# tnestmeyer/reflectance-filtering

Measured on AMD Instinct MI355X. Metric: megapixels/sec joint-bilateral sigma_c=20 sigma_s=22 @1080p, higher is better.
Workload: dtype f32

## Files before the change

reflectance_filtering_amd/csrc/rf_api.hip:

```cpp
#include "rf_common.hpp"

#include <atomic>
#include <cstring>

#include "reflectance_filtering_debug.h"

namespace rf {

void jbf_shutdown();
void cnn_shutdown();
void gf_shutdown();

char *last_error_buf()
{
    static thread_local char buf[512] = "";
    return buf;
}

int fail(int code, const char *fmt, ...)
{
    va_list ap;
    va_start(ap, fmt);
    vsnprintf(last_error_buf(), 512, fmt, ap);
    va_end(ap);
    return code;
}

static std::atomic<int> g_debug[kDbgCount];

int debug_get(int id) { return g_debug[id].load(std::memory_order_relaxed); }

}

extern "C" int rf_debug_option(const char *name, int value)
{
    static const char *const names[] = {"gf_two_kernel",     "jbf_stage_only",
                                                      "jbf_compiler_loop", "jbf_tile64_only",
                                                      "jbf_tune",          "jbf_f32_untiled",
                                                      "cnn_lds_columns",   "gf_seg_rows",
                                                      "gf_one_stream",     "gf_force_two_streams",
                                                      "gf_guide_cache",    "gf_chained",        "gf_no_compact",
                                                      "gf_exp_skip",       "gf_stagger",        "gf_parts",
                                                      "gf_s1_cap",         "gf_s1_min_wgs",
                                                      "jbf_lookahead1",    "gf_s1_legacy_strips",
                                                      "gf_exact_all_flagged", "gf_cw_chan_run",   "gf_exact"};
    static_assert(sizeof(names) / sizeof(names[0]) == rf::kDbgCount, "one name per DebugOption");
    if (name)
        for (int i = 0; i < rf::kDbgCount; i++)
            if (std::strcmp(name, names[i]) == 0)
                return rf::g_debug[i].exchange(value < 0 ? 0 : value);
    return rf::fail(RF_E_BADARG, "rf_debug_option: unknown option '%s'", name ? name : "(null)");
}

__global__ void clock_probe_kernel(unsigned long long *out, unsigned long long ticks)
{
    if (threadIdx.x != 0)
        return;
    const unsigned long long r0 = __builtin_amdgcn_s_memrealtime();
    const unsigned long long c0 = __builtin_amdgcn_s_memtime();
    unsigned long long r1 = r0;
    while (r1 - r0 < ticks) {
        __builtin_amdgcn_s_sleep(64);
        r1 = __builtin_amdgcn_s_memrealtime();
    }
    const unsigned long long c1 = __builtin_amdgcn_s_memtime();
    r1 = __builtin_amdgcn_s_memrealtime();
    out[0] = c1 - c0;
    out[1] = r1 - r0;
}

extern "C" int rf_debug_clock_probe(unsigned long long *out2, int micros, void *stream)
{
    if (!out2 || micros < 1 || micros > 1000000)
        return rf::fail(RF_E_BADARG, "rf_debug_clock_probe: bad argument");
    hipLaunchKernelGGL(clock_probe_kernel, dim3(1), dim3(64), 0, (hipStream_t)stream, out2,
                       (unsigned long long)micros * 100ull);
    RF_HIP_CHECK(hipGetLastError());
    return RF_OK;
}

#ifdef RF_GF_DEV_ONLY
extern "C" int rf_version(void) { return RF_VERSION | 0x40000000; }
#else
extern "C" int rf_version(void) { return RF_VERSION; }
#endif

#ifndef RF_TOOLCHAIN
#define RF_TOOLCHAIN "unknown toolchain"
#endif
extern "C" const char *rf_debug_build_info(void) { return RF_TOOLCHAIN; }

extern "C" const char *rf_last_error(void) { return rf::last_error_buf(); }

extern "C" int rf_shutdown(void)
{
    rf::jbf_shutdown();
    rf::cnn_shutdown();
    rf::gf_shutdown();
    return RF_OK;
}
```

reflectance_filtering_amd/csrc/rf_common.hpp:

```cpp
#pragma once
#include <hip/hip_runtime.h>

#include <cstdarg>
#include <cstdint>
#include <cstdio>

#include "reflectance_filtering.h"

namespace rf {

char *last_error_buf();
int fail(int code, const char *fmt, ...);

#define RF_HIP_CHECK(expr)                                                                   \
    do {                                                                                     \
        hipError_t _e = (expr);                                                              \
        if (_e != hipSuccess)                                                                \
            return ::rf::fail(RF_E_HIP, "%s failed: %s (%s:%d)", #expr, hipGetErrorString(_e), \
                              __FILE__, __LINE__);                                           \
    } while (0)

__host__ __device__ inline int border_interpolate(int p, int len, int border)
{
    if ((unsigned)p < (unsigned)len)
        return p;
    if (border == RF_BORDER_REPLICATE)
        return p < 0 ? 0 : len - 1;
    if (border == RF_BORDER_REFLECT || border == RF_BORDER_REFLECT_101) {
        const int delta = border == RF_BORDER_REFLECT_101;
        if (len == 1)
            return 0;
        do {
            p = p < 0 ? -p - 1 + delta : len - 1 - (p - len) - delta;
        } while ((unsigned)p >= (unsigned)len);
        return p;
    }
    if (border == RF_BORDER_WRAP) {
        if (p < 0)
            p -= ((p - len + 1) / len) * len;
        if (p >= len)
            p %= len;
        return p;
    }
    return -1;
}

__device__ inline uint8_t saturate_u8(float v)
{
    if (!(fabsf(v) < 2147483648.0f))
        return 0;
    int iv = __float2int_rn(v);
    iv = iv < 0 ? 0 : (iv > 255 ? 255 : iv);
    return (uint8_t)iv;
}

inline int ceil_div(int a, int b) { return (a + b - 1) / b; }

inline bool ranges_overlap(const void *a, size_t na, const void *b, size_t nb)
{
    const uintptr_t a0 = (uintptr_t)a, b0 = (uintptr_t)b;
    return a0 < b0 + nb && b0 < a0 + na;
}

enum DebugOption {
    kDbgGfTwoKernel = 0,
    kDbgJbfStageOnly,
    kDbgJbfCompilerLoop,
    kDbgJbfTile64Only,
    kDbgJbfTune,
    kDbgJbfF32Untiled,
    kDbgCnnLdsColumns,
    kDbgGfSegRows,
    kDbgGfOneStream,
    kDbgGfForceTwoStreams,
    kDbgGfGuideCache,
    kDbgGfChained,
    kDbgGfNoCompact,
    kDbgGfExpSkip,
    kDbgGfStagger,
    kDbgGfParts,
    kDbgGfS1Cap,
    kDbgGfS1MinWgs,
    kDbgJbfLookahead1,
    kDbgGfS1LegacyStrips,
    kDbgGfExactAllFlagged,
    kDbgGfCwChanRun,
    kDbgGfExact,
    kDbgCount
};
int debug_get(int id);

}
```

reflectance_filtering_amd/csrc/rf_jbf.hip:

```cpp
#include <atomic>
#include <cfloat>
#include <cmath>
#include <cstring>
#include <memory>
#include <mutex>
#include <type_traits>
#include <vector>

#include "rf_jbf_common.hpp"

namespace rf {

int jbf_colour_lut(int joint_cn, double sigma_color, std::vector<float> &lut)
{
    const double gauss_color_coeff = -0.5 / (sigma_color * sigma_color);
    const int nlut = 256 * joint_cn;
    lut.assign(nlut, 0.0f);
    for (int i = 0; i < nlut; i++)
        lut[i] = (float)std::exp(i * i * gauss_color_coeff);
    for (int i = 0; i < nlut; i++)
        if (lut[i] == 0.0f)
            return i + 1;
    return nlut;
}

void jbf_space_taps(int radius, double sigma_space, std::vector<int> &di, std::vector<int> &dj,
                    std::vector<float> &sw, std::vector<int> &hw)
{
    const double gauss_space_coeff = -0.5 / (sigma_space * sigma_space);
    di.clear();
    dj.clear();
    sw.clear();
    hw.assign(2 * radius + 1, -1);
    for (int i = -radius; i <= radius; i++)
        for (int j = -radius; j <= radius; j++) {
            double r = std::sqrt((double)i * i + (double)j * j);
            if (r > radius)
                continue;
            float wgt = (float)std::exp(r * r * gauss_space_coeff);
            di.push_back(i);
            dj.push_back(j);
            sw.push_back(wgt);
            if (j >= 0 && j > hw[i + radius])
                hw[i + radius] = j;
        }
}

namespace {

constexpr int kTileW = 64;
constexpr int kPix = 4;
constexpr int kMaxLds = 160 * 1024;
constexpr int kTlw2 = 144;
constexpr int kJbfMaxTiledR4 = 468;
constexpr int kJbfStageOnly = 0x1000, kJbfCompilerLoop = 0x2000, kJbfTile64Only = 0x4000;
constexpr int kJbfLookahead1 = 0x8000;

typedef uint32_t uint2v __attribute__((ext_vector_type(2)));
typedef float float4v __attribute__((ext_vector_type(4)));

struct JbfTables {
    int device = -1;
    int radius = 0;
    int joint_cn = 0;
    double sigma_color = 0, sigma_space = 0;
    int maxk = 0;
    int lut_len = 0;
    float *d_lut = nullptr;
    int *d_di = nullptr;
    int *d_dj = nullptr;
    float *d_sw = nullptr;
    int *d_hw = nullptr;
    int r4 = 0, sw_len = 0;
    float *d_swsym = nullptr;
    std::shared_ptr<void> keep;
};

struct CaptureRelax {
    hipStreamCaptureMode mode = hipStreamCaptureModeRelaxed;
    bool ok;
    CaptureRelax() { ok = hipThreadExchangeStreamCaptureMode(&mode) == hipSuccess; }
    ~CaptureRelax()
    {
        if (ok)
            (void)hipThreadExchangeStreamCaptureMode(&mode);
    }
};

struct JbfTableOwner {
    int device = 0;
    void *d_arena = nullptr;
    size_t bytes = 0;
    std::atomic<bool> pinned{false};
    ~JbfTableOwner()
    {
        int cur = 0;
        const bool switched = hipGetDevice(&cur) == hipSuccess && cur != device &&
                              hipSetDevice(device) == hipSuccess;
        if (d_arena)
            (void)hipFree(d_arena);
        if (switched)
            (void)hipSetDevice(cur);
    }
};

std::mutex g_mu;
std::vector<JbfTables> g_tables;
std::vector<std::shared_ptr<void>> g_retired;

bool stream_is_capturing(hipStream_t stream)
{
    hipStreamCaptureStatus cs = hipStreamCaptureStatusNone;
    if (hipStreamIsCapturing(stream, &cs) != hipSuccess) {
        (void)hipGetLastError();
        return false;
    }
    return cs != hipStreamCaptureStatusNone;
}

void drain_retired(hipStream_t stream)
{
    if (stream_is_capturing(stream))
        return;
    std::vector<std::shared_ptr<void>> bin;
    {
        std::lock_guard<std::mutex> lock(g_mu);
        bin.swap(g_retired);
    }
    if (!bin.empty()) {
        CaptureRelax relax;
        bin.clear();
    }
}

struct TablesHold {
    JbfTables &t;
    ~TablesHold()
    {
        if (t.keep && t.keep.use_count() == 1) {
            std::lock_guard<std::mutex> lock(g_mu);
            g_retired.push_back(std::move(t.keep));
        }
    }
};

void note_use_on(const JbfTables &t, hipStream_t stream)
{
    if (stream_is_capturing(stream))
        static_cast<JbfTableOwner *>(t.keep.get())->pinned.store(true, std::memory_order_relaxed);
}

int get_tables(int radius, int joint_cn, double sigma_color, double sigma_space, hipStream_t stream,
               JbfTables *out)
{
    int dev = 0;
    RF_HIP_CHECK(hipGetDevice(&dev));
    drain_retired(stream);
    {
        std::lock_guard<std::mutex> lock(g_mu);
        for (const JbfTables &t : g_tables)
            if (t.device == dev && t.radius == radius && t.joint_cn == joint_cn &&
                t.sigma_color == sigma_color && t.sigma_space == sigma_space) {
                *out = t;
                break;
            }
    }
    if (out->keep) {
        note_use_on(*out, stream);
        return RF_OK;
    }
    JbfTables t;
    t.device = dev;
    t.radius = radius;
    t.joint_cn = joint_cn;
    t.sigma_color = sigma_color;
    t.sigma_space = sigma_space;
    const int nlut = 256 * joint_cn;
    std::vector<float> lut;
    t.lut_len = jbf_colour_lut(joint_cn, sigma_color, lut);
    const int d = 2 * radius + 1;
    std::vector<int> di, dj, hw;
    std::vector<float> sw;
    jbf_space_taps(radius, sigma_space, di, dj, sw, hw);
    t.maxk = (int)di.size();
    t.r4 = (radius + 3) & ~3;
    t.sw_len = 2 * (t.r4 + 8);
    std::vector<float> swsym((size_t)(radius + 1) * t.sw_len, 0.0f);
    for (size_t k = 0; k < di.size(); k++)
        if (di[k] >= 0)
            swsym[(size_t)di[k] * t.sw_len + (t.r4 + 8) + dj[k]] = sw[k];
    const size_t part[6] = {sizeof(float) * swsym.size(), sizeof(float) * (size_t)nlut,
                            sizeof(int) * (size_t)t.maxk, sizeof(int) * (size_t)t.maxk,
                            sizeof(float) * (size_t)t.maxk, sizeof(int) * (size_t)d};
    const void *from[6] = {swsym.data(), lut.data(), di.data(), dj.data(), sw.data(), hw.data()};
    size_t off[6], total = 0;
    for (int k = 0; k < 6; k++) {
        off[k] = total;
        total += (part[k] + 255) & ~(size_t)255;
    }
    auto owner = std::make_shared<JbfTableOwner>();
    owner->device = dev;
    owner->bytes = total;
    t.keep = owner;
    {
        std::vector<char> image(total, 0);
        for (int k = 0; k < 6; k++)
            std::memcpy(image.data() + off[k], from[k], part[k]);
        CaptureRelax relax;
        hipStream_t ps = nullptr;
        RF_HIP_CHECK(hipStreamCreateWithFlags(&ps, hipStreamNonBlocking));
        struct StreamGuard {
            hipStream_t s;
            ~StreamGuard() { (void)hipStreamDestroy(s); }
        } guard{ps};
        RF_HIP_CHECK(hipMalloc(&owner->d_arena, total));
        RF_HIP_CHECK(hipMemcpyAsync(owner->d_arena, image.data(), total, hipMemcpyHostToDevice, ps));
        RF_HIP_CHECK(hipStreamSynchronize(ps));
    }
    char *db = static_cast<char *>(owner->d_arena);
    t.d_swsym = reinterpret_cast<float *>(db + off[0]);
    t.d_lut = reinterpret_cast<float *>(db + off[1]);
    t.d_di = reinterpret_cast<int *>(db + off[2]);
    t.d_dj = reinterpret_cast<int *>(db + off[3]);
    t.d_sw = reinterpret_cast<float *>(db + off[4]);
    t.d_hw = reinterpret_cast<int *>(db + off[5]);
    {
        std::lock_guard<std::mutex> lock(g_mu);
        bool found = false;
        for (const JbfTables &e : g_tables)
            if (e.device == dev && e.radius == radius && e.joint_cn == joint_cn &&
                e.sigma_color == sigma_color && e.sigma_space == sigma_space) {
                g_retired.push_back(std::move(t.keep));
                t = e;
                found = true;
                break;
            }
        if (!found) {
            if (g_tables.size() >= 64) {
                size_t victim = g_tables.size();
                for (size_t i = 0; i < g_tables.size(); i++) {
                    if (static_cast<JbfTableOwner *>(g_tables[i].keep.get())->pinned.load(
                            std::memory_order_relaxed))
                        continue;
                    if (victim == g_tables.size())
                        victim = i;
                    if (g_tables[i].device == dev) {
                        victim = i;
                        break;
                    }
                }
                if (victim != g_tables.size()) {
                    g_retired.push_back(std::move(g_tables[victim].keep));
                    g_tables.erase(g_tables.begin() + victim);
                }
            }
            g_tables.push_back(t);
        }
    }
    *out = t;
    note_use_on(*out, stream);
    return RF_OK;
}

__device__ inline void load_packed4(const uint8_t *img, size_t pix, int cn, uint32_t (&out)[4])
{
    const uint8_t *p = img + pix * (cn < 0 ? 1 : cn);
    if (cn == 3) {
        uint32_t d0, d1, d2;
        __builtin_memcpy(&d0, p, 4);
        __builtin_memcpy(&d1, p + 4, 4);
        __builtin_memcpy(&d2, p + 8, 4);
        out[0] = d0 & 0x00ffffffu;
        out[1] = (d0 >> 24) | ((d1 & 0xffffu) << 8);
        out[2] = (d1 >> 16) | ((d2 & 0xffu) << 16);
        out[3] = d2 >> 8;
    } else {
        uint32_t d0;
        __builtin_memcpy(&d0, p, 4);
        const uint32_t rep = cn < 0 ? 0x010101u : 1u;
        out[0] = (d0 & 0xffu) * rep;
        out[1] = ((d0 >> 8) & 0xffu) * rep;
        out[2] = ((d0 >> 16) & 0xffu) * rep;
        out[3] = (d0 >> 24) * rep;
    }
}

__device__ inline void load_tile_quad(const uint8_t *joint, const uint8_t *src, size_t img, int gy,
                                      int x_first, int w, int jcn, int scn, int border,
                                      uint32_t (&jv)[4], uint32_t (&sv)[4])
{
    if (gy < 0) {
#pragma unroll
        for (int u = 0; u < 4; u++)
            jv[u] = sv[u] = 0u;
        return;
    }
    const size_t row = img + (size_t)gy * w;
    if (x_first >= 0 && x_first + 3 < w) {
        load_packed4(joint, row + x_first, jcn, jv);
        load_packed4(src, row + x_first, scn, sv);
        return;
    }
#pragma unroll
    for (int u = 0; u < 4; u++) {
        const int gx = border_interpolate(x_first + u, w, border);
        jv[u] = gx < 0 ? 0u : load_packed(joint, row + gx, jcn);
        sv[u] = gx < 0 ? 0u : load_packed(src, row + gx, scn);
    }
}

__device__ inline int xcd_contiguous_tile(int b, int nblocks)
{
    const int per = nblocks >> 3;
    return b < (per << 3) ? (b & 7) * per + (b >> 3) : b;
}

__device__ inline float finish_value(float sum, float wsum_or_inv, int flags)
{
    return (flags & RF_JBF_TRUE_DIVISION) ? __fdiv_rn(sum, wsum_or_inv) : __fmul_rn(sum, wsum_or_inv);
}

template <int NCH_IN, int SCN>
__device__ inline void store_quad(uint8_t *dst, size_t img, int oy, int ox0, int h, int w,
                                  const float (&sum)[kPix][NCH_IN], const float (&wsum)[kPix],
                                  int flags)
{
    if (oy >= h || ox0 >= w)
        return;
    uint8_t px[kPix][3];
#pragma unroll
    for (int p = 0; p < kPix; p++) {
        const float d = (flags & RF_JBF_TRUE_DIVISION) ? wsum[p] : __fdiv_rn(1.0f, wsum[p]);
#pragma unroll
        for (int c = 0; c < SCN; c++)
            px[p][c] = saturate_u8(finish_value(sum[p][NCH_IN == 1 ? 0 : c], d, flags));
    }
    uint8_t *o = dst + (img + (size_t)oy * w + ox0) * SCN;
    if (SCN == 3 && ox0 + 3 < w) {
        uint32_t d[3];
        d[0] = px[0][0] | (px[0][1] << 8) | (px[0][2] << 16) | ((uint32_t)px[1][0] << 24);
        d[1] = px[1][1] | (px[1][2] << 8) | (px[2][0] << 16) | ((uint32_t)px[2][1] << 24);
        d[2] = px[2][2] | (px[3][0] << 8) | (px[3][1] << 16) | ((uint32_t)px[3][2] << 24);
        __builtin_memcpy(o, d, 12);
    } else if (SCN == 1 && ox0 + 3 < w) {
        const uint32_t d = px[0][0] | (px[1][0] << 8) | (px[2][0] << 16) | ((uint32_t)px[3][0] << 24);
        __builtin_memcpy(o, &d, 4);
    } else {
#pragma unroll
        for (int p = 0; p < kPix; p++)
            if (ox0 + p < w)
#pragma unroll
                for (int c = 0; c < SCN; c++)
                    o[p * SCN + c] = px[p][c];
    }
}

__global__ __launch_bounds__(256) void jbf_generic_kernel(
    const uint8_t *__restrict__ joint, const uint8_t *__restrict__ src, uint8_t *__restrict__ dst,
    int h, int w, int jcn, int scn, int border, const float *__restrict__ lut,
    const int *__restrict__ di, const int *__restrict__ dj, const float *__restrict__ sw, int maxk,
    int flags)
{
    const int x = blockIdx.x * 64 + (threadIdx.x & 63);
    const int y = blockIdx.y * 4 + (threadIdx.x >> 6);
    if (x >= w || y >= h)
        return;
    const size_t img = (size_t)blockIdx.z * h * w;
// ... 1093 lines not shown
            }
            __syncthreads();
            uint32_t jc[kPix];
#pragma unroll
            for (int p = 0; p < kPix; p++) {
                const int X = 4 * tx + p + r4;
                jc[p] = tile4[(ty + radius) * TLW + (X & 3) * Q4 + (X >> 2)] & 0x00ffffffu;
            }
            float sum[kPix][3], wsum[kPix];
#pragma unroll
            for (int p = 0; p < kPix; p++) {
                wsum[p] = 0.f;
                sum[p][0] = sum[p][1] = sum[p][2] = 0.f;
            }
            const uint32_t lut_lane_addr = lds_addr(lut_c) + (uint32_t)(tid & (CREP - 1)) * 4u;
            if (flags & kJbfCompilerLoop)
                jbf_tap_loop<3, CREP, false, TLW, 6>(lut_lane_addr, sw_addr0,
                                                     lds_addr(tile4) + (uint32_t)tx * 4u,
                                                     lds_addr(plane_b) + (uint32_t)tx * 2u, jc, 0u,
                                                     ty, radius, r4, sw_len, hwtab, sum, wsum);
            else
                jbf_tap_loop_rgb6<CREP, TLW>(lut_lane_addr, swsym,
                                             lds_addr(tile4) + (uint32_t)tx * 4u,
                                             lds_addr(plane_b) + (uint32_t)tx * 2u, jc, ty, radius,
                                             r4, sw_len, hwtab, sum, wsum);
            store_quad<3, 3>(dst, img, tile_y0 + ty, tile_x0 + 4 * tx, h, w, sum, wsum, flags);
            return;
        }
        if constexpr (TH != 64)
            return;
        float *lut_c = reinterpret_cast<float *>(smem + kT64Lds - nz * CREP * 4);
        const int tlh8 = crows + 2 * radius;
        uint16_t *plane_b = reinterpret_cast<uint16_t *>(tile_raw + (size_t)tlh8 * TLW * 4);
        for (int half = 0; half * crows < 64; half++) {
            const int y0 = tile_y0 + crows * half;
            if (y0 >= h)
                break;
            __syncthreads();
            if (half == 0)
                for (int i = tid; i < nz * CREP; i += NT)
                    lut_c[i] = lut[i / CREP];
            for (int item = tid; item < tlh8 * Q4; item += NT) {
                const int ry = item / Q4, k = item - ry * Q4;
                const int gy = border_interpolate(y0 - radius + ry, h, border);
                uint32_t jv[4], sv[4];
                load_tile_quad(joint, src, img, gy, tile_x0 - r4 + 4 * k, w, jcn, 3, border, jv, sv);
#pragma unroll
                for (int u = 0; u < 4; u++) {
                    tile4[ry * TLW + u * Q4 + k] = jv[u] | (sv[u] << 24);
                    plane_b[ry * TLW + u * Q4 + k] = (uint16_t)(sv[u] >> 8);
                }
            }
            __syncthreads();
            if (tid < 16 * crows) {
                uint32_t jc[kPix];
#pragma unroll
                for (int p = 0; p < kPix; p++) {
                    const int X = 4 * tx + p + r4;
                    jc[p] = tile4[(ty + radius) * TLW + (X & 3) * Q4 + (X >> 2)] & 0x00ffffffu;
                }
                float sum[kPix][3], wsum[kPix];
#pragma unroll
                for (int p = 0; p < kPix; p++) {
                    wsum[p] = 0.f;
                    sum[p][0] = sum[p][1] = sum[p][2] = 0.f;
                }
                const uint32_t lut_lane_addr = lds_addr(lut_c) + (uint32_t)(tid & (CREP - 1)) * 4u;
                if (flags & kJbfCompilerLoop)
                    jbf_tap_loop<3, CREP, false, TLW, 6>(lut_lane_addr, sw_addr0,
                                                         lds_addr(tile4) + (uint32_t)tx * 4u,
                                                         lds_addr(plane_b) + (uint32_t)tx * 2u, jc, 0u,
                                                         ty, radius, r4, sw_len, hwtab, sum, wsum);
                else
                    jbf_tap_loop_rgb6<CREP, TLW>(lut_lane_addr, swsym,
                                                 lds_addr(tile4) + (uint32_t)tx * 4u,
                                                 lds_addr(plane_b) + (uint32_t)tx * 2u, jc, ty, radius,
                                                 r4, sw_len, hwtab, sum, wsum);
                store_quad<3, 3>(dst, img, y0 + ty, tile_x0 + 4 * tx, h, w, sum, wsum, flags);
            }
        }
    }
}

__device__ inline void store_quad_channel(uint8_t *dst, size_t img, int oy, int ox0, int h, int w,
                                          int c, const float (&sum)[kPix][1],
                                          const float (&wsum)[kPix], int flags)
{
    if (oy >= h || ox0 >= w)
        return;
    uint8_t *o = dst + (img + (size_t)oy * w + ox0) * 3 + c;
#pragma unroll
    for (int p = 0; p < kPix; p++) {
        if (ox0 + p >= w)
            break;
        const float d = (flags & RF_JBF_TRUE_DIVISION) ? wsum[p] : __fdiv_rn(1.0f, wsum[p]);
        o[p * 3] = saturate_u8(finish_value(sum[p][0], d, flags));
    }
}

__global__ void lds_oob_probe_kernel(uint32_t *out)
{
    extern __shared__ __align__(16) unsigned char smem[];
    uint32_t *w = reinterpret_cast<uint32_t *>(smem);
    for (int i = threadIdx.x; i < kT64Lds / 4; i += blockDim.x)
        w[i] = 0xdeadbeefu;
    __syncthreads();
    uint32_t bad = 0;
    const uint32_t addrs[4] = {(uint32_t)kT64Lds + 4u * threadIdx.x, (uint32_t)kT64Lds + 61056u,
                               262140u, (uint32_t)kT64Lds - 4u};
#pragma unroll
    for (int k = 0; k < 4; k++) {
        uint32_t v;
        asm volatile("ds_read_b32 %0, %1\n s_waitcnt lgkmcnt(0)" : "=v"(v) : "v"(addrs[k]));
        bad |= (k < 3) ? (v != 0u) : (v != 0xdeadbeefu);
    }
    if (bad)
        atomicOr(out, 1u);
}

struct Tiled2Config {
    int th, lutrep;
    bool full_lut;
};

size_t tiled2_lds_bytes(const JbfTables &t, int th, int lutrep, bool full_lut)
{
    const int lut_len = full_lut ? 256 * t.joint_cn : t.lut_len;
    const size_t lut_bytes = ((size_t)lut_len * lutrep * 4 + 15) & ~(size_t)15;
    const size_t sw_bytes = ((size_t)(t.radius + 1) * t.sw_len * 4 + 15) & ~(size_t)15;
    return 16 + lut_bytes + sw_bytes + (size_t)kTlw2 * (th + 2 * t.radius) * sizeof(uint2);
}

template <int SCN, int TH, int LUTREP>
int launch_tiled2(const JbfTables &t, bool full_lut, const uint8_t *joint, const uint8_t *src,
                  uint8_t *dst, int n, int h, int w, int jcn, int border, int flags,
                  hipStream_t stream)
{
    const int lut_len = full_lut ? 256 * t.joint_cn : t.lut_len;
    const bool clamp = lut_len < 256 * t.joint_cn;
    const size_t lds = tiled2_lds_bytes(t, TH, LUTREP, full_lut);
    const int tiles_x = ceil_div(w, kTileW), tiles_y = ceil_div(h, TH);
    const long long blocks = (long long)tiles_x * tiles_y * n;
    if (blocks > 0x7fffffffLL)
        return fail(RF_E_UNSUPPORTED, "rf_jbf_u8: batch too large for one launch");
    auto kern = clamp ? jbf_tiled2_kernel<SCN, TH, LUTREP, true>
                      : jbf_tiled2_kernel<SCN, TH, LUTREP, false>;
    RF_HIP_CHECK(hipFuncSetAttribute((const void *)kern, hipFuncAttributeMaxDynamicSharedMemorySize,
                                     (int)lds));
    hipLaunchKernelGGL(kern, dim3((unsigned)blocks), dim3(16 * TH), lds, stream, joint, src, dst, h,
                       w, jcn, t.radius, border, t.d_lut, lut_len, t.d_hw, t.d_swsym, t.sw_len,
                       tiles_x, tiles_x * tiles_y, flags);
    return RF_OK;
}


std::vector<int> g_oob_ok;

int lds_oob_reads_zero(int dev, bool *ok)
{
    {
        std::lock_guard<std::mutex> lock(g_mu);
        if ((int)g_oob_ok.size() <= dev)
            g_oob_ok.resize(dev + 1, -1);
        if (g_oob_ok[dev] >= 0) {
            *ok = g_oob_ok[dev] == 1;
            return RF_OK;
        }
    }
    CaptureRelax relax;
    uint32_t *d_flag = nullptr;
    hipStream_t ps = nullptr;
    RF_HIP_CHECK(hipStreamCreateWithFlags(&ps, hipStreamNonBlocking));
    struct StreamGuard {
        hipStream_t s;
        ~StreamGuard() { (void)hipStreamDestroy(s); }
    } guard{ps};
    RF_HIP_CHECK(hipMalloc(&d_flag, sizeof(uint32_t)));
    RF_HIP_CHECK(hipMemsetAsync(d_flag, 0, sizeof(uint32_t), ps));
    RF_HIP_CHECK(hipFuncSetAttribute((const void *)lds_oob_probe_kernel,
                                     hipFuncAttributeMaxDynamicSharedMemorySize, kT64Lds));
    hipLaunchKernelGGL(lds_oob_probe_kernel, dim3(8), dim3(256), kT64Lds, ps, d_flag);
    uint32_t flag = 1;
    RF_HIP_CHECK(hipMemcpyAsync(&flag, d_flag, sizeof(flag), hipMemcpyDeviceToHost, ps));
    RF_HIP_CHECK(hipStreamSynchronize(ps));
    (void)hipFree(d_flag);
    std::lock_guard<std::mutex> lock(g_mu);
    g_oob_ok[dev] = flag == 0 ? 1 : 0;
    *ok = flag == 0;
    return RF_OK;
}

int tile64_fits(const JbfTables &t, int nz, int grep, int crep, int scn, int tlw, int th, int flags)
{
    if (2 * t.r4 + 4 * (1024 / th) + 8 > tlw)
        return 0;
    const bool need_sw = (flags & (kJbfCompilerLoop | kJbfLookahead1)) != 0;
    const size_t sw_bytes =
        16 + (need_sw ? ((size_t)(t.radius + 1) * t.sw_len * 4 + 15) & ~(size_t)15 : 0);
    const size_t grey = sw_bytes + (size_t)tlw * (th + 2 * t.radius) * 4 + (size_t)nz * grep * 4;
    if (grey > (size_t)kT64Lds)
        return 0;
    if (scn == 1)
        return 32;
    if (sw_bytes + (size_t)tlw * (th + 2 * t.radius) * 6 + (size_t)nz * crep * 4 <= (size_t)kT64Lds)
        return th;
    if (th != 64)
        return 0;
    for (int crows = 32; crows >= 8; crows >>= 1) {
        const size_t col =
            sw_bytes + (size_t)tlw * (crows + 2 * t.radius) * 6 + (size_t)nz * crep * 4;
        if (col <= (size_t)kT64Lds)
            return crows;
    }
    return 0;
}

template <int SCN, int GREP, int CREP, int TLW, int TH = 64>
int launch_tile64(const JbfTables &t, int nz, int crows, const uint8_t *joint, const uint8_t *src,
                  uint8_t *dst, int n, int h, int w, int jcn, int border, int flags,
                  hipStream_t stream, int y_base = 0, int rows = -1, int x_base = 0, int cols = -1)
{
    if (rows < 0)
        rows = h;
    if (cols < 0)
        cols = w;
    const int tiles_x = ceil_div(cols, 4 * (1024 / TH)), tiles_y = ceil_div(rows, TH);
    const long long blocks = (long long)tiles_x * tiles_y * n;
    if (blocks > 0x7fffffffLL)
        return fail(RF_E_UNSUPPORTED, "rf_jbf_u8: batch too large for one launch");
    auto kern = jbf_tile64_kernel<SCN, GREP, CREP, TLW, TH>;
    RF_HIP_CHECK(hipFuncSetAttribute((const void *)kern, hipFuncAttributeMaxDynamicSharedMemorySize,
                                     kT64Lds));
    hipLaunchKernelGGL(kern, dim3((unsigned)blocks), dim3(1024), kT64Lds, stream, joint, src, dst,
                       h, w, jcn, t.radius, border, t.d_lut, nz, t.d_hw, t.d_swsym, t.sw_len,
                       tiles_x, tiles_x * tiles_y, flags, crows, y_base, x_base);
    return RF_OK;
}

template <int SCN, int GREP, int CREP>
int launch_tile64_rows(const JbfTables &t, int nz, int crows, const uint8_t *joint,
                       const uint8_t *src, uint8_t *dst, int n, int h, int w, int jcn, int border,
                       int flags, hipStream_t stream)
{
    const bool only64 = (flags & kJbfTile64Only) != 0;
    int sx = 0;
    if (SCN == 1 && !only64 && (w & 63) > 0 && (w & 63) <= 32 &&
        tile64_fits(t, nz, GREP, CREP, SCN, 136, 128, flags) > 0 && ceil_div(h, 128) < ceil_div(h, 64))
        sx = w & 63;
    const int cols_main = w - sx;
    const int rem = h & 63;
    const bool ok32 = tile64_fits(t, nz, GREP, CREP, SCN, 208, 32, flags) > 0;
    const bool ok16 = SCN == 1 && tile64_fits(t, nz, GREP, CREP, SCN, 336, 16, flags) > 0;
    int s32 = 0, s16 = 0;
    if (rem > 0 && rem <= 16 && ok16)
        s16 = rem;
    else if (rem > 0 && rem <= 32 && ok32)
        s32 = rem;
    else if (rem > 32 && rem <= 48 && ok32 && ok16)
        s32 = 32, s16 = rem - 32;
    const int strip_blocks =
        (s32 ? ceil_div(cols_main, 128) : 0) + (s16 ? ceil_div(cols_main, 256) : 0);
    if (only64 || cols_main == 0 || ((s32 || s16) && strip_blocks >= ceil_div(cols_main, 64)))
        s32 = s16 = 0;
    const int rows_main = h - s32 - s16;
    int rc = RF_OK;
    if (rows_main > 0 && cols_main > 0)
        rc = launch_tile64<SCN, GREP, CREP, 144>(t, nz, crows, joint, src, dst, n, h, w, jcn,
                                                 border, flags, stream, 0, rows_main, 0, cols_main);
    if (rc == RF_OK && s32)
        rc = launch_tile64<SCN, GREP, CREP, 208, 32>(t, nz, 32, joint, src, dst, n, h, w, jcn,
                                                     border, flags, stream, rows_main, s32, 0,
                                                     cols_main);
    if constexpr (SCN == 1) {
        if (rc == RF_OK && s16)
            rc = launch_tile64<1, GREP, CREP, 336, 16>(t, nz, 32, joint, src, dst, n, h, w, jcn,
                                                       border, flags, stream, rows_main + s32, s16,
                                                       0, cols_main);
        if (rc == RF_OK && sx)
            rc = launch_tile64<1, GREP, CREP, 136, 128>(t, nz, 32, joint, src, dst, n, h, w, jcn,
                                                        border, flags, stream, 0, h, cols_main, sx);
    }
    return rc;
}

template <int GREP, int TLW>
__global__ __launch_bounds__(1024) void jbf_slab_kernel(
    const uint8_t *__restrict__ joint, const uint8_t *__restrict__ src, uint8_t *__restrict__ dst,
    int h, int w, int jcn, int scn, int radius, int border, const float *__restrict__ lut, int nz,
    const int *__restrict__ hwtab, const float *__restrict__ swsym, int sw_len, int tiles_x,
    int tiles_per_img, int flags, int crows_g, int slab_g, int crows_c, int slab_c)
{
    constexpr int NT = 1024, Q4 = TLW / 4, QW = 16;
    static_assert(TLW % 32 == 16, "row pitch keeps the rows of a half-wave on disjoint banks");
    extern __shared__ __align__(16) unsigned char smem[];
    int *flag_word = reinterpret_cast<int *>(smem);
    uint32_t *tile4 = reinterpret_cast<uint32_t *>(smem + 16);
    const int tid = threadIdx.x;
    if (tid == 0)
        *flag_word = 3;
    const int tile_id = xcd_contiguous_tile((int)blockIdx.x, (int)gridDim.x);
    const int img_idx = tile_id / tiles_per_img;
    const int t_in_img = tile_id - img_idx * tiles_per_img;
    const int tile_y0 = (t_in_img / tiles_x) * 64;
    const int tile_x0 = (t_in_img % tiles_x) * 64;
    const size_t img = (size_t)img_idx * h * w;
    const int r4 = (radius + 3) & ~3;
    const int tx = tid % QW, ty = tid / QW;
    float *lut_g = reinterpret_cast<float *>(smem + kT64Lds - nz * GREP * 4);
    for (int i = tid; i < nz * GREP; i += NT)
        lut_g[i] = lut[i / GREP];
    const uint32_t lut_lane_addr = lds_addr(lut_g) + (uint32_t)(tid & (GREP - 1)) * 4u;
    const uint32_t tile_lane_addr = lds_addr(tile4) + (uint32_t)tx * 4u;
    int all_grey = scn == 1;
    if (scn == 3) {
        int grey = 1;
        const int rows_all = min(64, h - tile_y0) + 2 * radius;
        for (int item = tid; item < rows_all * Q4; item += NT) {
            const int ry = item / Q4, k = item - ry * Q4;
            const int gy = border_interpolate(tile_y0 - radius + ry, h, border);
            uint32_t jv[4], sv[4];
            load_tile_quad(joint, src, img, gy, tile_x0 - r4 + 4 * k, w, jcn, scn, border, jv, sv);
#pragma unroll
            for (int u = 0; u < 4; u++)
                grey &= (int)(((sv[u] ^ (sv[u] >> 8)) & 0xffffu) == 0u);
        }
        all_grey = __builtin_amdgcn_readfirstlane(block_all2(grey, 1, flag_word) & 1);
    }
    const bool rgb6 = !all_grey && crows_c > 0;
    const int crows = rgb6 ? crows_c : crows_g, slab_rows = rgb6 ? slab_c : slab_g;
    const bool active = tid < QW * crows;
    for (int y0 = tile_y0; y0 < tile_y0 + 64 && y0 < h; y0 += crows) {
        for (int c = 0; c < (all_grey || rgb6 ? 1 : scn); c++) {
            uint32_t jc[kPix];
            float sum1[kPix][1], sum3[kPix][3], wsum[kPix];
            {
                uint32_t jv[4], sv[4];
                load_tile_quad(joint, src, img, min(y0 + ty, h - 1), tile_x0 + 4 * tx, w, jcn, scn, border,
                               jv, sv);
#pragma unroll
                for (int p = 0; p < kPix; p++) {
                    jc[p] = jv[p] & 0x00ffffffu;
                    sum1[p][0] = sum3[p][0] = sum3[p][1] = sum3[p][2] = 0.f;
                    wsum[p] = 0.f;
                }
            }
            for (int i0 = -radius; i0 <= radius; i0 += slab_rows) {
                const int i1 = min(i0 + slab_rows - 1, radius);
                const int tlh = crows + (i1 - i0);
                uint16_t *plane_b = reinterpret_cast<uint16_t *>(tile4 + (size_t)tlh * TLW);
                __syncthreads();
                for (int item = tid; item < tlh * Q4; item += NT) {
                    const int ry = item / Q4, k = item - ry * Q4;
                    const int gy = border_interpolate(y0 + i0 + ry, h, border);
                    uint32_t jv[4], sv[4];
                    load_tile_quad(joint, src, img, gy, tile_x0 - r4 + 4 * k, w, jcn, scn, border, jv, sv);
#pragma unroll
                    for (int u = 0; u < 4; u++) {
                        tile4[ry * TLW + u * Q4 + k] = jv[u] | (((sv[u] >> (8 * c)) & 0xffu) << 24);
                        if (rgb6)
                            plane_b[ry * TLW + u * Q4 + k] = (uint16_t)(sv[u] >> 8);
                    }
                }
                __syncthreads();
                if (active) {
                    if (rgb6)
                        jbf_tap_loop_rgb6<GREP, TLW, true>(lut_lane_addr, swsym, tile_lane_addr,
                                                           lds_addr(plane_b) + (uint32_t)tx * 2u, jc, ty,
                                                           radius, r4, sw_len, hwtab, sum3, wsum, i0, i1, -i0);
                    else
                        jbf_tap_loop_grey4_la2<GREP, TLW, false, true>(lut_lane_addr, swsym, tile_lane_addr,
                                                                       jc, ty, radius, r4, sw_len, hwtab,
                                                                       sum1, wsum, i0, i1, -i0);
                }
            }
            if (active) {
                if (rgb6)
                    store_quad<3, 3>(dst, img, y0 + ty, tile_x0 + 4 * tx, h, w, sum3, wsum, flags);
                else if (scn == 1)
                    store_quad<1, 1>(dst, img, y0 + ty, tile_x0 + 4 * tx, h, w, sum1, wsum, flags);
                else if (all_grey)
                    store_quad<1, 3>(dst, img, y0 + ty, tile_x0 + 4 * tx, h, w, sum1, wsum, flags);
                else
// ... 224 lines not shown
                for (int ch = 0; ch < SCN; ch++)
                    sum[p][ch] = __fadd_rn(sum[p][ch], __fmul_rn(wgt, st[u][ch]));
                wsum[p] = __fadd_rn(wsum[p], wgt);
            }
            w3 = w2;
            w2 = w1;
            w1 = w0;
            w0 = wn[u];
        }
    };
    auto rows = [&](auto interior_c) __attribute__((always_inline)) {
        constexpr bool INTERIOR = decltype(interior_c)::value;
        for (int i = -radius; i <= radius; i++) {
            const int hw = hwtab[i + radius];
            const int hw4 = (hw + 3) & ~3;
            const int yy = INTERIOR ? y + i : border_interpolate(y + i, h, border);
            const float *jrow = joint + (img + (size_t)yy * w) * JCN;
            const float *srow = src + (img + (size_t)yy * w) * SCN;
            const float *wrow = sw_s + (i < 0 ? -i : i) * sw_len + (r4 + 8);
            float w0 = wrow[-hw4], w1 = wrow[-hw4 - 1], w2 = wrow[-hw4 - 2], w3 = wrow[-hw4 - 3];
            for (int c4 = -hw4; c4 <= hw4; c4 += 4) {
                if (c4 - 3 >= -hw && c4 + 3 <= hw)
                    group(interior_c, std::false_type{}, jrow, srow, wrow, c4, hw, w0, w1, w2, w3);
                else
                    group(interior_c, std::true_type{}, jrow, srow, wrow, c4, hw, w0, w1, w2, w3);
            }
        }
    };
    if (interior)
        rows(std::true_type{});
    else
        rows(std::false_type{});
    if (ty0 + ly >= h)
        return;
#pragma unroll
    for (int p = 0; p < 4; p++) {
        if (x0 + p >= w)
            continue;
        const float inv = __fdiv_rn(1.0f, wsum[p]);
#pragma unroll
        for (int c = 0; c < SCN; c++)
            dst[(img + (size_t)y * w + x0 + p) * SCN + c] = __fmul_rn(sum[p][c], inv);
    }
}

}

void jbf_shutdown()
{
    std::lock_guard<std::mutex> lock(g_mu);
    g_tables.clear();
    g_retired.clear();
}

}

extern "C" int rf_jbf_u8(const uint8_t *joint, const uint8_t *src, uint8_t *dst, int n, int h,
                         int w, int joint_cn, int src_cn, int d, double sigma_color,
                         double sigma_space, int border, int flags, void *stream_)
{
    using namespace rf;
    if (n == 0)
        return RF_OK;
    if (!joint || !src || !dst)
        return fail(RF_E_BADARG, "rf_jbf_u8: NULL image pointer");
    if (n < 0 || h <= 0 || w <= 0)
        return fail(RF_E_BADARG, "rf_jbf_u8: bad size n=%d h=%d w=%d", n, h, w);
    if ((joint_cn != 1 && joint_cn != 3) || (src_cn != 1 && src_cn != 3))
        return fail(RF_E_UNSUPPORTED, "rf_jbf_u8: channels must be 1 or 3 (joint %d, src %d)",
                    joint_cn, src_cn);
    if (border < 0 || border > 4)
        return fail(RF_E_UNSUPPORTED, "rf_jbf_u8: border type %d", border);
    {
        const size_t px = (size_t)n * h * w;
        if (ranges_overlap(dst, px * src_cn, joint, px * joint_cn) ||
            ranges_overlap(dst, px * src_cn, src, px * src_cn))
            return fail(RF_E_BADARG, "rf_jbf_u8: dst must not overlap an input");
    }
    if (flags & ~(RF_JBF_TRUE_DIVISION | RF_JBF_FORCE_GENERIC | RF_JBF_GREY_AS_BGR))
        return fail(RF_E_BADARG, "rf_jbf_u8: unknown flag bits 0x%x", flags);
    flags |= (debug_get(kDbgJbfStageOnly) ? kJbfStageOnly : 0) |
             (debug_get(kDbgJbfCompilerLoop) ? kJbfCompilerLoop : 0) |
             (debug_get(kDbgJbfTile64Only) ? kJbfTile64Only : 0) |
             (debug_get(kDbgJbfLookahead1) ? kJbfLookahead1 : 0);
    if (sigma_color <= 0)
        sigma_color = 1;
    if (sigma_space <= 0)
        sigma_space = 1;
    int radius = d <= 0 ? (int)std::lrint(sigma_space * 1.5) : d / 2;
    if (radius < 1)
        radius = 1;
    if (radius > 4096)
        return fail(RF_E_UNSUPPORTED, "rf_jbf_u8: radius %d too large", radius);
    hipStream_t stream = (hipStream_t)stream_;
    const int joint_cn_arg = joint_cn;
    if ((flags & RF_JBF_GREY_AS_BGR) && joint_cn == 1)
        joint_cn = 3;
    const int jcn_kernel = joint_cn_arg == 1 && joint_cn == 3 ? -1 : joint_cn;
    JbfTables t;
    TablesHold hold{t};
    int rc = get_tables(radius, joint_cn, sigma_color, sigma_space, stream, &t);
    if (rc != RF_OK)
        return rc;

    const int tune = debug_get(kDbgJbfTune) & 0xf;
    static const Tiled2Config kCfg[] = {{48, 16, false}, {32, 8, true},  {32, 32, false},
                                        {32, 16, false}, {64, 16, false}, {48, 8, false}};
    constexpr int kNumCfg = (int)(sizeof(kCfg) / sizeof(kCfg[0]));
    bool done = false;
    if (!(flags & RF_JBF_FORCE_GENERIC) && t.r4 <= kJbfMaxTiledR4 && (tune == 0 || tune == 7)) {
        bool oob_ok = false;
        rc = lds_oob_reads_zero(t.device, &oob_ok);
        if (rc != RF_OK)
            return rc;
        const int nz = t.lut_len < 256 * joint_cn ? t.lut_len - 1 : t.lut_len;
        if (oob_ok) {
#define RF_T64(G_, C_, W_)                                                                        \
    if (!done && (min_rows < 64 || C_ >= 8) &&                                                    \
        tile64_fits(t, nz, G_, C_, src_cn, W_, 64, flags) >= min_rows) {                          \
        const int crows_ = tile64_fits(t, nz, G_, C_, src_cn, W_, 64, flags);                     \
        if (W_ == 144)                                                                            \
            rc = src_cn == 3 ? launch_tile64_rows<3, G_, C_>(t, nz, crows_, joint, src, dst, n,   \
                                                             h, w, jcn_kernel, border, flags,     \
                                                             stream)                              \
                             : launch_tile64_rows<1, G_, C_>(t, nz, crows_, joint, src, dst, n,   \
                                                             h, w, jcn_kernel, border, flags,     \
                                                             stream);                             \
        else                                                                                      \
            rc = src_cn == 3 ? launch_tile64<3, G_, C_, W_>(t, nz, crows_, joint, src, dst, n, h, \
                                                            w, jcn_kernel, border, flags, stream) \
                             : launch_tile64<1, G_, C_, W_>(t, nz, crows_, joint, src, dst, n, h, \
                                                            w, jcn_kernel, border, flags, stream);\
        if (rc != RF_OK)                                                                          \
            return rc;                                                                            \
        done = true;                                                                              \
    }
            for (int min_rows = src_cn == 3 ? 64 : 1; min_rows >= 1 && !done;
                 min_rows = min_rows == 64 ? 1 : 0) {
                RF_T64(32, 32, 144)
                RF_T64(32, 16, 144)
                RF_T64(16, 8, 144)
                RF_T64(8, 4, 144)
                RF_T64(32, 16, 176)
                RF_T64(32, 8, 176)
                RF_T64(32, 4, 176)
                RF_T64(16, 8, 176)
                RF_T64(8, 4, 176)
            }
#undef RF_T64
            if (!done && t.r4 > 52 && t.r4 <= kJbfMaxTiledR4) {
                const int tlw = t.r4 <= 68    ? 208
                                : t.r4 <= 84  ? 240
                                : t.r4 <= 100 ? 272
                                : t.r4 <= 116 ? 304
                                : t.r4 <= 132 ? 336
                                : t.r4 <= 164 ? 400
                                : t.r4 <= 212 ? 496
                                : t.r4 <= 276 ? 624
                                : t.r4 <= 372 ? 816
                                              : 1008;
                int crows = 0, slab = 0, rep = 0, crows_c = 0, slab_c = 0;
                for (int g : {16, 8}) {
                    int cr, sl;
                    slab_fits(t, nz, g, tlw, 4, &cr, &sl);
                    if (cr > crows)
                        crows = cr, slab = sl, rep = g;
                }
// ... 233 lines not shown
```

Measured before the change: 2188.

## Add persistent tile64 JBF kernel that prefetches the next tile during taps

Adds a persistent variant of the 64-row tile kernel, launched with one workgroup per CU. Each workgroup walks a contiguous range of tiles grouped by XCD, and issues the global loads for the next tile's halo into registers before running the current tile's tap loop. After the taps it unpacks those registers into LDS. This is meant to hide global load latency and cut launch and LUT-setup cost per tile. The trade-offs are more register pressure, only one 1024-thread workgroup per CU, and possible load imbalance. It is on by default through a new debug option, and it also adds a __syncthreads in the slab kernel after the flag initialisation.

Result: no change. 2202 (median of 6 runs) (+0.6%).

```diff
diff --git a/reflectance_filtering_amd/csrc/rf_api.hip b/reflectance_filtering_amd/csrc/rf_api.hip
--- a/reflectance_filtering_amd/csrc/rf_api.hip
+++ b/reflectance_filtering_amd/csrc/rf_api.hip
@@ -27,6 +27,7 @@
 }
 
 static std::atomic<int> g_debug[kDbgCount];
+[[maybe_unused]] static const bool g_debug_defaults =(g_debug[kDbgJbfPersistent].store(1), true);
 
 int debug_get(int id) { return g_debug[id].load(std::memory_order_relaxed); }
 
@@ -43,7 +44,8 @@
                                                       "gf_exp_skip",       "gf_stagger",        "gf_parts",
                                                       "gf_s1_cap",         "gf_s1_min_wgs",
                                                       "jbf_lookahead1",    "gf_s1_legacy_strips",
-                                                      "gf_exact_all_flagged", "gf_cw_chan_run",   "gf_exact"};
+                                                      "gf_exact_all_flagged", "gf_cw_chan_run",   "gf_exact",
+                                                      "jbf_persistent"};
     static_assert(sizeof(names) / sizeof(names[0]) == rf::kDbgCount, "one name per DebugOption");
     if (name)
         for (int i = 0; i < rf::kDbgCount; i++)
diff --git a/reflectance_filtering_amd/csrc/rf_common.hpp b/reflectance_filtering_amd/csrc/rf_common.hpp
--- a/reflectance_filtering_amd/csrc/rf_common.hpp
+++ b/reflectance_filtering_amd/csrc/rf_common.hpp
@@ -86,6 +86,7 @@
     kDbgGfExactAllFlagged,
     kDbgGfCwChanRun,
     kDbgGfExact,
+    kDbgJbfPersistent,
     kDbgCount
 };
 int debug_get(int id);
diff --git a/reflectance_filtering_amd/csrc/rf_jbf.hip b/reflectance_filtering_amd/csrc/rf_jbf.hip
--- a/reflectance_filtering_amd/csrc/rf_jbf.hip
+++ b/reflectance_filtering_amd/csrc/rf_jbf.hip
@@ -55,12 +55,14 @@
 constexpr int kJbfMaxTiledR4 = 468;
 constexpr int kJbfStageOnly = 0x1000, kJbfCompilerLoop = 0x2000, kJbfTile64Only = 0x4000;
 constexpr int kJbfLookahead1 = 0x8000;
+constexpr int kJbfOneTilePerWg = 0x10000;
 
 typedef uint32_t uint2v __attribute__((ext_vector_type(2)));
 typedef float float4v __attribute__((ext_vector_type(4)));
 
 struct JbfTables {
     int device = -1;
+    int num_cu = 0;
     int radius = 0;
     int joint_cn = 0;
     double sigma_color = 0, sigma_space = 0;
@@ -171,6 +173,7 @@
     }
     JbfTables t;
     t.device = dev;
+    RF_HIP_CHECK(hipDeviceGetAttribute(&t.num_cu, hipDeviceAttributeMultiprocessorCount, dev));
     t.radius = radius;
     t.joint_cn = joint_cn;
     t.sigma_color = sigma_color;
@@ -262,27 +265,43 @@
     return RF_OK;
 }
 
+template <int N>
+__device__ inline void load_raw4(const uint8_t *img, size_t pix, int cn, uint32_t (&d)[N])
+{
+    const uint8_t *p = img + pix * (cn < 0 ? 1 : cn);
+    __builtin_memcpy(&d[0], p, 4);
+    if constexpr (N == 3) {
+        if (cn == 3) {
+            __builtin_memcpy(&d[1], p + 4, 4);
+            __builtin_memcpy(&d[2], p + 8, 4);
+        }
+    }
+}
+
+template <int N>
+__device__ inline void unpack_raw4(const uint32_t (&d)[N], int cn, uint32_t (&out)[4])
+{
+    if constexpr (N == 3) {
+        if (cn == 3) {
+            out[0] = d[0] & 0x00ffffffu;
+            out[1] = (d[0] >> 24) | ((d[1] & 0xffffu) << 8);
+            out[2] = (d[1] >> 16) | ((d[2] & 0xffu) << 16);
+            out[3] = d[2] >> 8;
+            return;
+        }
+    }
+    const uint32_t rep = cn < 0 ? 0x010101u : 1u;
+    out[0] = (d[0] & 0xffu) * rep;
+    out[1] = ((d[0] >> 8) & 0xffu) * rep;
+    out[2] = ((d[0] >> 16) & 0xffu) * rep;
+    out[3] = (d[0] >> 24) * rep;
+}
+
 __device__ inline void load_packed4(const uint8_t *img, size_t pix, int cn, uint32_t (&out)[4])
 {
-    const uint8_t *p = img + pix * (cn < 0 ? 1 : cn);
-    if (cn == 3) {
-        uint32_t d0, d1, d2;
-        __builtin_memcpy(&d0, p, 4);
-        __builtin_memcpy(&d1, p + 4, 4);
-        __builtin_memcpy(&d2, p + 8, 4);
-        out[0] = d0 & 0x00ffffffu;
-        out[1] = (d0 >> 24) | ((d1 & 0xffffu) << 8);
-        out[2] = (d1 >> 16) | ((d2 & 0xffu) << 16);
-        out[3] = d2 >> 8;
-    } else {
-        uint32_t d0;
-        __builtin_memcpy(&d0, p, 4);
-        const uint32_t rep = cn < 0 ? 0x010101u : 1u;
-        out[0] = (d0 & 0xffu) * rep;
-        out[1] = ((d0 >> 8) & 0xffu) * rep;
-        out[2] = ((d0 >> 16) & 0xffu) * rep;
-        out[3] = (d0 >> 24) * rep;
-    }
+    uint32_t d[3];
+    load_raw4(img, pix, cn, d);
+    unpack_raw4(d, cn, out);
 }
 
 __device__ inline void load_tile_quad(const uint8_t *joint, const uint8_t *src, size_t img, int gy,
@@ -1542,6 +1561,306 @@
     }
 }
 
+template <int SCN, int GREP, int CREP, int TLW, int TH = 64>
+__global__ __launch_bounds__(1024) void jbf_tile64_persistent_kernel(
+    const uint8_t *__restrict__ joint, const uint8_t *__restrict__ src, uint8_t *__restrict__ dst,
+    int h, int w, int jcn, int radius, int border, const float *__restrict__ lut, int nz,
+    const int *__restrict__ hwtab, const float *__restrict__ swsym, int sw_len, int tiles_x,
+    int tiles_per_img, int flags, int crows, int y_base, int x_base, int ntiles)
+{
+    constexpr int NT = 1024;
+    constexpr int QW = NT / TH;
+    constexpr int TW = 4 * QW;
+    static_assert(TH == 64 || TH == 32 || ((TH == 16 || TH == 128) && SCN == 1), "tile shapes");
+    static_assert(QW >= 32 || (QW == 16 && TLW % 32 == 16) || (QW == 8 && TLW % 32 == 8),
+                  "row pitch keeps the rows of a half-wave on disjoint banks");
+    constexpr int Q4 = TLW / 4;
+    constexpr int NS = SCN == 3 ? 3 : 1;
+    constexpr int PF = SCN == 1 ? 5 : 3;
+    constexpr int PFC = 1;
+    extern __shared__ __align__(16) unsigned char smem[];
+    int *flag_words = reinterpret_cast<int *>(smem);
+    const bool need_sw = (flags & (kJbfCompilerLoop | kJbfLookahead1)) != 0;
+    float *swl = reinterpret_cast<float *>(smem + 16);
+    const int sw_bytes = need_sw ? ((radius + 1) * sw_len * 4 + 15) & ~15 : 0;
+    unsigned char *tile_raw = smem + 16 + sw_bytes;
+    const int tid = threadIdx.x;
+    const int r4 = (radius + 3) & ~3;
+    const int tx = tid % QW;
+    const int ty = tid / QW;
+    const int tlh = TH + 2 * radius;
+    const int n_items = tlh * Q4;
+
+    int tile, tile_end, tile_step;
+    {
+        const int nwg = (int)gridDim.x, b = (int)blockIdx.x;
+        const int nx = nwg < 8 ? nwg : 8;
+        const int xcd = b % nx, q = nwg / nx, rem = nwg % nx;
+        const int before = xcd * q + (xcd < rem ? xcd : rem);
+        tile_step = q + (xcd < rem ? 1 : 0);
+        tile = (int)((long long)ntiles * before / nwg) + b / nx;
+        tile_end = (int)((long long)ntiles * (before + tile_step) / nwg);
+    }
+    if (tile >= tile_end)
+        return;
+    auto tile_origin = [&](int t, size_t &img_out, int &y0_out, int &x0_out) {
+        const int img_idx = t / tiles_per_img;
+        const int t_in_img = t - img_idx * tiles_per_img;
+        y0_out = y_base + (t_in_img / tiles_x) * TH;
+        x0_out = x_base + (t_in_img % tiles_x) * TW;
+        img_out = (size_t)img_idx * h * w;
+    };
+
+    if (tid == 0)
+        flag_words[0] = flag_words[1] = 3;
+    if (need_sw)
+        for (int i = tid; i < (radius + 1) * sw_len; i += NT)
+            swl[i] = swsym[i];
+    float *lut_g = reinterpret_cast<float *>(smem + kT64Lds - nz * GREP * 4);
+    float *lut_c = reinterpret_cast<float *>(smem + kT64Lds - nz * CREP * 4);
+    for (int i = tid; i < nz * GREP; i += NT)
+        lut_g[i] = lut[i / GREP];
+    int lut_kind = 0;
+    __syncthreads();
+
+    uint32_t *tile4 = reinterpret_cast<uint32_t *>(tile_raw);
+    const bool j1_ok = !(flags & kJbfCompilerLoop);
+    const bool j1 = SCN == 1 && jcn != 3 && j1_ok;
+    const uint32_t j1_scale = (uint32_t)(jcn == 1 ? 1 : 3) * (GREP * 4u);
+    int grey = 1, grey_joint = 1;
+    auto write_item = [&](int item, const uint32_t (&jv)[4], const uint32_t (&sv)[4]) {
+        const int ry = item / Q4, k = item - ry * Q4;
+#pragma unroll
+        for (int u = 0; u < 4; u++) {
+            if (SCN == 3)
+                grey &= (int)(((sv[u] ^ (sv[u] >> 8)) & 0xffffu) == 0u);
+            if (jcn == 3)
+                grey_joint &= (int)(((jv[u] ^ (jv[u] >> 8)) & 0xffffu) == 0u);
+            const uint32_t jfield = j1 ? (jv[u] & 0xffu) * j1_scale : jv[u];
+            tile4[ry * TLW + u * Q4 + k] = jfield | (sv[u] << 24);
+        }
+    };
+    auto stage_item = [&](int item, size_t img, int tile_y0, int tile_x0) {
+        const int ry = item / Q4, k = item - ry * Q4;
+        const int gy = border_interpolate(tile_y0 - radius + ry, h, border);
+        uint32_t jv[4], sv[4];
+        load_tile_quad(joint, src, img, gy, tile_x0 - r4 + 4 * k, w, jcn, SCN, border, jv, sv);
+        write_item(item, jv, sv);
+    };
+
+    size_t img;
+    int tile_y0, tile_x0;
+    tile_origin(tile, img, tile_y0, tile_x0);
+    for (int item = tid; item < n_items; item += NT)
+        stage_item(item, img, tile_y0, tile_x0);
+
+    for (int n = 0;; n++) {
+        const int grey_bits =
+            __builtin_amdgcn_readfirstlane(block_all2(grey, grey_joint, flag_words + (n & 1)));
+        if (tid == 0)
+            flag_words[(n & 1) ^ 1] = 3;
+        const int all_grey = grey_bits & 1;
+        const int next = tile + tile_step;
+        const bool has_next = next < tile_end;
+        size_t nimg = 0;
+        int ny0 = 0, nx0 = 0;
+        if (has_next)
+            tile_origin(next, nimg, ny0, nx0);
+        const bool j1_late = !j1 && j1_ok && (SCN == 1 || all_grey) && (grey_bits & 2);
+        if (j1_late) {
+            for (int idx = tid; idx < tlh * TLW; idx += NT) {
+                const uint32_t t = tile4[idx];
+                tile4[idx] = (t & 0xffu) * j1_scale | (t & 0xff000000u);
+            }
+            __syncthreads();
+        }
+
+        uint32_t jraw[PF][3], sraw[PF][NS];
+        uint32_t pf_have = 0;
+        int tid_tile = tid;
+        asm volatile("" : "+v"(tid_tile));
+        auto prefetch = [&](auto rounds_c) {
+#pragma unroll
+            for (int r = 0; r < decltype(rounds_c)::value; r++) {
+                const int item = tid_tile + r * NT;
+                if (!has_next || item >= n_items)
+                    continue;
+                const int ry = item / Q4, k = item - ry * Q4;
+                const int gy = border_interpolate(ny0 - radius + ry, h, border);
+                const int xf = nx0 - r4 + 4 * k;
+                if (gy >= 0 && xf >= 0 && xf + 3 < w) {
+                    const size_t pix = nimg + (size_t)gy * w + xf;
+                    load_raw4(joint, pix, jcn, jraw[r]);
+                    load_raw4(src, pix, SCN, sraw[r]);
+                    pf_have |= 1u << r;
+                }
+            }
+        };
+
+        const uint32_t sw_addr0 = lds_addr(swl);
+        const bool taps = !(flags & kJbfStageOnly);
+        if (SCN == 1 || all_grey) {
+            if (CREP != GREP && lut_kind != 0) {
+                for (int i = tid; i < nz * GREP; i += NT)
+                    lut_g[i] = lut[i / GREP];
+                lut_kind = 0;
+                __syncthreads();
+            }
+            prefetch(std::integral_constant<int, PF>{});
+            if (taps) {
+                uint32_t jc[kPix];
+#pragma unroll
+                for (int p = 0; p < kPix; p++) {
+                    const int X = 4 * tx + p + r4;
+                    jc[p] = tile4[(ty + radius) * TLW + (X & 3) * Q4 + (X >> 2)] & 0x00ffffffu;
+                }
+                float sum1[kPix][1], wsum[kPix];
+#pragma unroll
+                for (int p = 0; p < kPix; p++) {
+                    sum1[p][0] = 0.f;
+                    wsum[p] = 0.f;
+                }
+                const uint32_t lut_lane_addr = lds_addr(lut_g) + (uint32_t)(tid & (GREP - 1)) * 4u;
+                const uint32_t tile_lane_addr = lds_addr(tile4) + (uint32_t)tx * 4u;
+                if (flags & kJbfCompilerLoop)
+                    jbf_tap_loop<1, GREP, false, TLW, 4>(lut_lane_addr, sw_addr0, tile_lane_addr, 0u, jc,
+                                                         0u, ty, radius, r4, sw_len, hwtab, sum1, wsum);
+                else if (flags & kJbfLookahead1) {
+                    if (j1 || j1_late)
+                        jbf_tap_loop_grey4<GREP, TLW, true>(lut_lane_addr, sw_addr0, tile_lane_addr, jc,
+                                                            ty, radius, r4, sw_len, hwtab, sum1, wsum);
+                    else
+                        jbf_tap_loop_grey4<GREP, TLW>(lut_lane_addr, sw_addr0, tile_lane_addr, jc, ty,
+                                                      radius, r4, sw_len, hwtab, sum1, wsum);
+                } else if (j1 || j1_late)
+                    jbf_tap_loop_grey4_la2<GREP, TLW, true>(lut_lane_addr, swsym, tile_lane_addr, jc, ty,
+                                                            radius, r4, sw_len, hwtab, sum1, wsum);
+                else
+                    jbf_tap_loop_grey4_la2<GREP, TLW>(lut_lane_addr, swsym, tile_lane_addr, jc, ty,
+                                                      radius, r4, sw_len, hwtab, sum1, wsum);
+                store_quad<1, SCN>(dst, img, tile_y0 + ty, tile_x0 + 4 * tx, h, w, sum1, wsum, flags);
+            }
+        } else if constexpr (SCN == 3) {
+            if (CREP != GREP && lut_kind != 1) {
+                __syncthreads();
+                for (int i = tid; i < nz * CREP; i += NT)
+                    lut_c[i] = lut[i / CREP];
+                lut_kind = 1;
+            }
+            if (crows == TH) {
+                uint16_t *plane_b = reinterpret_cast<uint16_t *>(tile_raw + (size_t)tlh * TLW * 4);
+                for (int item = tid; item < n_items; item += NT) {
+                    const int ry = item / Q4, k = item - ry * Q4;
+                    const int gy = border_interpolate(tile_y0 - radius + ry, h, border);
+                    uint32_t jv[4], sv[4];
+                    load_tile_quad(joint, src, img, gy, tile_x0 - r4 + 4 * k, w, jcn, 3, border, jv, sv);
+#pragma unroll
+                    for (int u = 0; u < 4; u++)
+                        plane_b[ry * TLW + u * Q4 + k] = (uint16_t)(sv[u] >> 8);
+                }
+                __syncthreads();
+                prefetch(std::integral_constant<int, PFC>{});
+                if (taps) {
+                    uint32_t jc[kPix];
+#pragma unroll
+                    for (int p = 0; p < kPix; p++) {
+                        const int X = 4 * tx + p + r4;
+                        jc[p] = tile4[(ty + radius) * TLW + (X & 3) * Q4 + (X >> 2)] & 0x00ffffffu;
+                    }
+                    float sum[kPix][3], wsum[kPix];
+#pragma unroll
+                    for (int p = 0; p < kPix; p++) {
+                        wsum[p] = 0.f;
+                        sum[p][0] = sum[p][1] = sum[p][2] = 0.f;
+                    }
+                    const uint32_t lut_lane_addr = lds_addr(lut_c) + (uint32_t)(tid & (CREP - 1)) * 4u;
+                    if (flags & kJbfCompilerLoop)
+                        jbf_tap_loop<3, CREP, false, TLW, 6>(lut_lane_addr, sw_addr0,
+                                                             lds_addr(tile4) + (uint32_t)tx * 4u,
+                                                             lds_addr(plane_b) + (uint32_t)tx * 2u, jc,
+                                                             0u, ty, radius, r4, sw_len, hwtab, sum, wsum);
+                    else
+                        jbf_tap_loop_rgb6<CREP, TLW>(lut_lane_addr, swsym,
+                                                     lds_addr(tile4) + (uint32_t)tx * 4u,
+                                                     lds_addr(plane_b) + (uint32_t)tx * 2u, jc, ty,
+                                                     radius, r4, sw_len, hwtab, sum, wsum);
+                    store_quad<3, 3>(dst, img, tile_y0 + ty, tile_x0 + 4 * tx, h, w, sum, wsum, flags);
+                }
+            } else if constexpr (TH == 64) {
+                const int tlh8 = crows + 2 * radius;
+                uint16_t *plane_b = reinterpret_cast<uint16_t *>(tile_raw + (size_t)tlh8 * TLW * 4);
+                for (int half = 0; half * crows < 64; half++) {
+                    const int y0 = tile_y0 + crows * half;
+                    if (y0 >= h)
+                        break;
+                    __syncthreads();
+                    for (int item = tid; item < tlh8 * Q4; item += NT) {
+                        const int ry = item / Q4, k = item - ry * Q4;
+                        const int gy = border_interpolate(y0 - radius + ry, h, border);
+                        uint32_t jv[4], sv[4];
+                        load_tile_quad(joint, src, img, gy, tile_x0 - r4 + 4 * k, w, jcn, 3, border, jv, sv);
+#pragma unroll
+                        for (int u = 0; u < 4; u++) {
+                            tile4[ry * TLW + u * Q4 + k] = jv[u] | (sv[u] << 24);
+                            plane_b[ry * TLW + u * Q4 + k] = (uint16_t)(sv[u] >> 8);
+                        }
+                    }
+                    __syncthreads();
+                    if (taps && tid < 16 * crows) {
+                        uint32_t jc[kPix];
+#pragma unroll
+                        for (int p = 0; p < kPix; p++) {
+                            const int X = 4 * tx + p + r4;
+                            jc[p] = tile4[(ty + radius) * TLW + (X & 3) * Q4 + (X >> 2)] & 0x00ffffffu;
+                        }
+                        float sum[kPix][3], wsum[kPix];
+#pragma unroll
+                        for (int p = 0; p < kPix; p++) {
+                            wsum[p] = 0.f;
+                            sum[p][0] = sum[p][1] = sum[p][2] = 0.f;
+                        }
+                        const uint32_t lut_lane_addr =
+                            lds_addr(lut_c) + (uint32_t)(tid & (CREP - 1)) * 4u;
+                        if (flags & kJbfCompilerLoop)
+                            jbf_tap_loop<3, CREP, false, TLW, 6>(
+                                lut_lane_addr, sw_addr0, lds_addr(tile4) + (uint32_t)tx * 4u,
+                                lds_addr(plane_b) + (uint32_t)tx * 2u, jc, 0u, ty, radius, r4, sw_len,
+                                hwtab, sum, wsum);
+                        else
+                            jbf_tap_loop_rgb6<CREP, TLW>(lut_lane_addr, swsym,
+                                                         lds_addr(tile4) + (uint32_t)tx * 4u,
+                                                         lds_addr(plane_b) + (uint32_t)tx * 2u, jc, ty,
+                                                         radius, r4, sw_len, hwtab, sum, wsum);
+                        store_quad<3, 3>(dst, img, y0 + ty, tile_x0 + 4 * tx, h, w, sum, wsum, flags);
+                    }
+                }
+            }
+        }
+        if (!has_next)
+            break;
+
+        __syncthreads();
+        tile = next;
+        img = nimg;
+        tile_y0 = ny0;
+        tile_x0 = nx0;
+        grey = grey_joint = 1;
+        asm volatile("" : "+v"(tid_tile));
+#pragma unroll
+        for (int r = 0; r < PF; r++) {
+            if (pf_have & (1u << r)) {
+                uint32_t jv[4], sv[4];
+                unpack_raw4(jraw[r], jcn, jv);
+                unpack_raw4(sraw[r], SCN, sv);
+                write_item(tid_tile + r * NT, jv, sv);
+            }
+        }
+        for (int item = tid_tile, r = 0; item < n_items; item += NT, r++)
+            if (r >= PF || !((pf_have >> r) & 1u))
+                stage_item(item, img, tile_y0, tile_x0);
+    }
+}
+
 __device__ inline void store_quad_channel(uint8_t *dst, size_t img, int oy, int ox0, int h, int w,
                                           int c, const float (&sum)[kPix][1],
                                           const float (&wsum)[kPix], int flags)
@@ -1688,6 +2007,16 @@
     const long long blocks = (long long)tiles_x * tiles_y * n;
     if (blocks > 0x7fffffffLL)
         return fail(RF_E_UNSUPPORTED, "rf_jbf_u8: batch too large for one launch");
+    if (!(flags & kJbfOneTilePerWg)) {
+        auto pkern = jbf_tile64_persistent_kernel<SCN, GREP, CREP, TLW, TH>;
+        const long long wgs = blocks < t.num_cu ? blocks : (long long)t.num_cu;
+        RF_HIP_CHECK(hipFuncSetAttribute((const void *)pkern,
+                                         hipFuncAttributeMaxDynamicSharedMemorySize, kT64Lds));
+        hipLaunchKernelGGL(pkern, dim3((unsigned)wgs), dim3(1024), kT64Lds, stream, joint, src, dst,
+                           h, w, jcn, t.radius, border, t.d_lut, nz, t.d_hw, t.d_swsym, t.sw_len,
+                           tiles_x, tiles_x * tiles_y, flags, crows, y_base, x_base, (int)blocks);
+        return RF_OK;
+    }
     auto kern = jbf_tile64_kernel<SCN, GREP, CREP, TLW, TH>;
     RF_HIP_CHECK(hipFuncSetAttribute((const void *)kern, hipFuncAttributeMaxDynamicSharedMemorySize,
                                      kT64Lds));
@@ -1758,6 +2087,7 @@
     const int tid = threadIdx.x;
     if (tid == 0)
         *flag_word = 3;
+    __syncthreads();
     const int tile_id = xcd_contiguous_tile((int)blockIdx.x, (int)gridDim.x);
     const int img_idx = tile_id / tiles_per_img;
     const int t_in_img = tile_id - img_idx * tiles_per_img;
@@ -2148,7 +2478,8 @@
     flags |= (debug_get(kDbgJbfStageOnly) ? kJbfStageOnly : 0) |
              (debug_get(kDbgJbfCompilerLoop) ? kJbfCompilerLoop : 0) |
              (debug_get(kDbgJbfTile64Only) ? kJbfTile64Only : 0) |
-             (debug_get(kDbgJbfLookahead1) ? kJbfLookahead1 : 0);
+             (debug_get(kDbgJbfLookahead1) ? kJbfLookahead1 : 0) |
+             (debug_get(kDbgJbfPersistent) ? 0 : kJbfOneTilePerWg);
     if (sigma_color <= 0)
         sigma_color = 1;
     if (sigma_space <= 0)
```
